# TimD1/vcfdist

Hardware: AMD Instinct MI355X
Metric: supercluster-alignments/sec (higher is better)
Workload: dtype int32; 1 GPU; wgs_synth; superclusters_per_gpu=1000000, span_dist=lognormal(median 20, sigma 1.2) clip [4,10000]

## Files before the change

vcfdist_amd/csrc/pr_api.hip:

```cpp
#include <hip/hip_runtime.h>
#include <hip/hip_ext.h>
#include <dlfcn.h>

#include <algorithm>
#include <atomic>
#include <chrono>
#include <cstdarg>
#include <cstdio>
#include <cstdlib>
#include <cstring>
#include <condition_variable>
#include <deque>
#include <functional>
#include <mutex>
#include <string>
#include <thread>
#include <tuple>
#include <unordered_map>
#include <unordered_set>
#include <vector>

#include "../../include/vcfdist_pr.h"
#include "pr_device.h"
#include "pr_plan.h"
// ... 935 lines not shown
    for (int k = 0; k < 2; k++)
        if (hipEventCreateWithFlags(&h->ev_cred[k], hipEventDisableTiming) != hipSuccess) return fail(nullptr, VPR_ERR_DEVICE, "hipEventCreate failed");
    if (const char *e = getenv("VPR_LONG_LT")) { const int v = atoi(e); if (v >= 64 && v <= 2048) h->long_lt = v; }
    memset(&h->dB, 0, sizeof(h->dB));
    memset(&h->timing, 0, sizeof(h->timing));
    const char *prio_map = exp_getenv("VPR_STREAM_PRIO");
    if (prio_map && strlen(prio_map) != size_t(N_CLASSES + 5)) prio_map = nullptr;
    if (hipSetDevice(cfg->device) != hipSuccess) { delete h; return fail(nullptr, VPR_ERR_DEVICE, "hipSetDevice failed"); }
    int prio_lo = 0, prio_hi = 0;
    (void)hipDeviceGetStreamPriorityRange(&prio_lo, &prio_hi);
    auto prio_of = [&](int idx, int dflt) { return !prio_map ? dflt : (prio_map[idx] == 'h' ? prio_hi : (prio_map[idx] == 'l' ? prio_lo : (prio_hi + prio_lo) / 2)); };
    if (hipStreamCreateWithPriority(&h->stream, exp_getenv("VPR_MAIN_BLOCKING") ? hipStreamDefault : hipStreamNonBlocking, prio_of(N_CLASSES + 4, (prio_hi + prio_lo) / 2)) != hipSuccess) {
        delete h;
        return fail(nullptr, VPR_ERR_DEVICE, "hipStreamCreate failed");
    }
    {
        size_t free_b = 0, total_b = 0;
        if (hipMemGetInfo(&free_b, &total_b) != hipSuccess) { delete h; return fail(nullptr, VPR_ERR_DEVICE, "hipMemGetInfo failed"); }
        h->dev_total = int64_t(total_b);
        h->tie_scratch_max = std::max<int64_t>(h->dev_total / 16, int64_t(64) << 20);
        h->lad_arena_max = std::max<int64_t>(h->dev_total / 8, int64_t(64) << 20);
    }
    if (const char *e = exp_getenv("VPR_STREAM_PAD")) {
        static std::atomic<int> n_handles{0};
        const int me = n_handles.fetch_add(1);
        const char *p = e;
        for (int i = 0; i < me && p; i++) { p = strchr(p, ','); if (p) p++; }
        if (p) {
            const int n_lo = atoi(p);
            const char *c = strchr(p, ':');
// ... 351 lines not shown
                h->res_dev = base; h->res_bytes = off;
            }
        }
    }
    if ((rc = dev_alloc(h, &R.tally, 6))) return rc;
    R.max_qual = h->cfg.max_qual;
    R.credit_threshold = h->cfg.credit_threshold;
    R.phase_threshold = h->cfg.phase_threshold;
    h->tie_list_cap = int32_t(std::min<size_t>(std::max<size_t>(na, 4096), size_t(1) << 20));
    if ((rc = dev_alloc(h, &h->d_tie_list, size_t(h->tie_list_cap)))) return rc;
    if ((rc = dev_alloc(h, &h->d_tie_cnt, 8))) return rc;
    if ((rc = dev_alloc(h, &h->d_tie_ndec, TIE_DEC_SLOTS))) return rc;
    const size_t n_fail = 4 * na + na / 16 + 1024, n_slots = 2 + 4 * LadderCtx::N_SLOTS;
    if ((rc = dev_alloc(h, &h->d_fail, n_fail))) return rc;
    if ((rc = dev_alloc(h, &h->d_cnt, n_slots))) return rc;
    {
        void *pf = nullptr, *pc = nullptr, *pl = nullptr, *pt = nullptr;
        { int rc_pin = pin_alloc(h, &pf, n_fail * sizeof(int32_t)); if (rc_pin) return rc_pin; }
        { int rc_pin = pin_alloc(h, &pc, n_slots * sizeof(int32_t)); if (rc_pin) return rc_pin; }
        { int rc_pin = pin_alloc(h, &pl, size_t(h->tie_list_cap) * sizeof(int4)); if (rc_pin) return rc_pin; }
        { int rc_pin = pin_alloc(h, &pt, 32 * sizeof(int32_t)); if (rc_pin) return rc_pin; }
        h->hp_fail = static_cast<int32_t *>(pf);
        h->hp_cnt = static_cast<int32_t *>(pc);
        h->hp_tie_list = static_cast<int4 *>(pl);
        h->hp_tie_cnt = static_cast<int32_t *>(pt);
        h->hp_flag = h->hp_tie_cnt + 8;
        memset(h->hp_cnt, 0, n_slots * sizeof(int32_t));
        memset(h->hp_tie_cnt, 0, 32 * sizeof(int32_t));
    }

// ... 313 lines not shown
    }
    double phase_ms[6] = {0, 0, 0, 0, 0, 0};
    void phase(int k) { phase_ms[k] = std::chrono::duration<double, std::milli>(std::chrono::steady_clock::now() - call0).count(); }
    void lapx(const char *what) {
        if (h->debug) fprintf(stderr, "[vpr] execute %-34s %8.3f ms\n", what,
                              std::chrono::duration<double, std::milli>(std::chrono::steady_clock::now() - wall0).count());
    }

    void post_flag(int idx, hipStream_t ks) {
        flag_exp[idx] = ++h->flag_seq;
        hipLaunchKernelGGL(k_flag, dim3(1), dim3(1), 0, ks, h->hp_flag + idx, flag_exp[idx]);
        const hipError_t e = hipGetLastError();
        if (e != hipSuccess && launch_err == hipSuccess) launch_err = e;
    }
    hipError_t launch_err = hipSuccess;
    int64_t zl_wave0 = 0, zl_rows = 0;

    int idle_check(int64_t idle_polls, std::chrono::steady_clock::time_point since) {
        if (launch_err != hipSuccess) return fail(h, VPR_ERR_DEVICE, "kernel launch failed: %s", hipGetErrorString(launch_err));
        if (idle_polls % 2048) return VPR_OK;
        hipStream_t ss[] = {h->stream, h->cls_stream[0], h->cls_stream[1], h->cls_stream[2], h->cls_stream[3], h->cls_stream[4],
                            h->cls_stream[5], h->cls_stream[6], h->cls_stream[7],
                            h->tie_stream[0], h->tie_stream[1], h->tie_stream[2], h->tie_stream[3]};
        bool busy = false;
        for (hipStream_t s_ : ss) {
            const hipError_t e = hipStreamQuery(s_);
            if (e != hipSuccess && e != hipErrorNotReady) return fail(h, VPR_ERR_DEVICE, "stream error while waiting for a round: %s", hipGetErrorString(e));
            busy = busy || e == hipErrorNotReady;
        }
        const double idle_s = std::chrono::duration<double>(std::chrono::steady_clock::now() - since).count();
// ... 407 lines not shown
            }
        }
        return VPR_OK;
    }

    int enqueue_part(const Plan &P, const int32_t *d_work, int64_t off, int32_t cnt, int lv, hipStream_t ks,
                            int slot, int64_t fail_off, bool long_part, int64_t part_cells, int64_t part_in,
                            int64_t part_dense, int dtag_override = -1, int phases = 7,
                            const int32_t *n_dev = nullptr, int32_t n_all = 0, int tag_or = 0) {
        const int W = LV_WINDOW[lv], C = W / 64, tag = LV_TAG[lv] | tag_or;
        const bool q16 = lv <= LV_Q16, zero = lv == LV_Z;
        const int dtag = dtag_override >= 0 ? dtag_override : tag;
        const int32_t *list = d_work + off;
        int32_t *a_i32 = reinterpret_cast<int32_t *>(P.arena);
        PathEnt *a_path = reinterpret_cast<PathEnt *>(P.arena);
        vpr_launch_stat ls;
        memset(&ls, 0, sizeof(ls));
        ls.threads = q16 ? 16 : 64; ls.cells_per_thread = q16 ? 1 : C; ls.n_units = cnt;
        ls.cells = part_cells;
        ls.cells_dense = part_dense;
        ls.bytes_algorithmic = ls.cells + part_in;
        int rc = VPR_OK;
        if (phases & 1) {
        if (zero) {
            ls.bytes_algorithmic = 36 * zl_rows;
            ls.cells = 8 * zl_rows;
        }
        cells_touched += ls.cells;
        const bool save = lv == LV_C1 && !tag_or && fwd_save_delta != 0;
        RestoreJob *rjobs = nullptr;
// ... 7 lines not shown
                const auto it = tie_early.find(P.work[size_t(off) + size_t(k)]);
                if (it == tie_early.end() || it->second.plan != &h->plan0 || (it->second.mode != 1 && it->second.mode != 3) ||
                    it->second.pos < tie_resident->work_off || it->second.pos >= tie_resident->work_off + tie_resident->n_long) { restore = false; break; }
                const AlnDesc od = plan_desc(h, h->plan0, size_t(it->second.pos)), nd = plan_desc(h, P, size_t(off) + size_t(k));
                if (od.band_pad != LV_TAG[LV_C1] || od.pitch[0] != nd.pitch[0] || od.pitch[1] != nd.pitch[1] ||
                    od.mat_off[1] + int64_t(od.pitch[1]) * od.Lt > h->save_bytes) { restore = false; break; }
                rjobs[k] = RestoreJob{{od.mat_off[0], od.mat_off[1]}, od.blo_off};
            }
        }
        rc = timed(1, ls, ks, restore ? "k_restore_stripe" : band_fwd_name(lv), [&] {
            if (zero)
                hipExtLaunchKernelGGL(k_zero_lane, dim3((cnt + 63) / 64), dim3(64), h->zl_lds_bytes, ks, own_a, own_b, 0, h->d_descs, list, cnt,
                                      h->d_zl_hdr + zl_wave0, h->d_zl_in, h->d_zl_log, h->d_outs, a_path,
                                      (h->cfg.flags & VPR_CFG_KEEP_PATHS) ? 1 : 0, h->d_d1_hdr ? h->d1_max_rows : 0, h->lane_prio_rows);
            else if (q16)
                hipLaunchKernelGGL(k_fwd_q16, dim3((cnt + 3) / 4), dim3(64), 0, ks, h->dB, h->d_descs, list, cnt,
                                   P.arena, a_i32, h->d_outs, n_dev);
            else if (restore)
                hipLaunchKernelGGL(k_restore_stripe, dim3(cnt), dim3(256), 0, ks, h->d_descs, list, rjobs, h->plan0.arena,
                                   int64_t(reinterpret_cast<intptr_t>(h->d_save) - reinterpret_cast<intptr_t>(h->plan0.arena)), P.arena, a_i32);
            else if (save)
                hipLaunchKernelGGL(k_fwd_stripe_save, dim3(cnt), dim3(64), 0, ks, h->dB, h->d_descs, list, P.arena, a_i32, h->d_outs,
                                   fwd_save_delta);
            else
                hipLaunchKernelGGL(band_fwd_kernel(lv), dim3(cnt), dim3(lv >= LV_C4 ? W : 64), 0,
                                   ks, h->dB, h->d_descs, list, P.arena, a_i32, h->d_outs);
            hipLaunchKernelGGL(k_fwd_band_finish, dim3((cnt + 255) / 256), dim3(256), 0, ks, list, cnt, h->d_outs, tag, n_dev);
        }, zero);
        if (rc) return rc;
        n_fwd++;
        {
            const int32_t nc = n_dev ? n_all : cnt;
            if (zero && h->d_d1_blk) ordered_fails(list, nc, h->d_fail + fail_off, h->d_cnt + slot, n_dev, ks);
            else
            hipLaunchKernelGGL(k_collect_fails, dim3((nc + 255) / 256), dim3(256), 0, ks, list, nc, h->d_outs,
                               h->d_fail + fail_off, h->d_cnt + slot, zero ? 1 : 0, n_dev);
            hipLaunchKernelGGL(k_publish_fails, dim3(zero ? 1 : std::min((nc + 255) / 256, 1024)), dim3(256), 0, ks,
                               h->d_fail + fail_off, h->d_cnt + slot, h->hp_fail + fail_off, h->hp_cnt + slot, zero ? 0 : 1);
        }
        HIPCHK(h, hipEventRecord(h->ev_slot[slot], ks));
        }
        if ((phases & 2) && !zero) {
        ls.bytes_algorithmic = ls.cells;
        rc = timed(2, ls, ks, band_bwd_name(lv), [&] {
            if (q16)
                hipLaunchKernelGGL(k_bwd_q16, dim3((cnt + 3) / 4), dim3(64), 0, ks, h->dB, h->d_descs, list, cnt,
                                   P.arena, a_i32, h->d_outs, tag, dtag, n_dev);
            else
                hipLaunchKernelGGL(band_bwd_kernel(lv), dim3(cnt), dim3(lv >= LV_C4 ? W : 64), 0,
                                   ks, h->dB, h->d_descs, list, P.arena, a_i32, h->d_outs, tag);
        });
        if (rc) return rc;
        }
        if (!(phases & 4)) return rc;
        const bool wave_walk = !q16 && (long_part || cnt < 2048);
        int64_t walk_rows_sum = 0;
        if (lv == LV_C1 && !h->seq_walk)
            for (int32_t k = 0; k < cnt && walk_rows_sum <= WSEG_MAX_ROWS; k++) walk_rows_sum += plan_desc(h, P, size_t(off) + size_t(k)).Lt;
        const bool seg_walk = lv == LV_C1 && !h->seq_walk && walk_rows_sum <= WSEG_MAX_ROWS;
        const bool row_walk = lv == LV_C1 && (wave_walk || seg_walk);
        vpr_launch_stat ws_;
        memset(&ws_, 0, sizeof(ws_));
        ws_.threads = q16 ? 16 : 64; ws_.n_units = cnt; ws_.cells_per_thread = 2;
        if (q16) {
            if (!zero) rc = timed(3, ws_, ks, "k_walk_q16", [&] {
                hipLaunchKernelGGL(k_walk_q16, dim3((cnt + 3) / 4), dim3(64), 0, ks, h->dB, h->d_descs, list, cnt,
                                   P.arena, a_i32, h->d_outs, a_path, tag, dtag, n_dev);
            });
            if (rc) return rc;
            ws_.cells_per_thread = 3;
            if (zero) ws_.bytes_algorithmic = 20 * zl_rows;
            if (zero) rc = timed(3, ws_, ks, "k_zero_tail", [&] {
                hipLaunchKernelGGL(k_zero_tail, dim3((cnt + 63) / 64), dim3(64), 0, ks, h->dB, h->d_descs, list, cnt, h->d_zl_hdr + zl_wave0,
                                   h->d_zl_in, h->d_zl_log, h->d_outs, a_path, (h->cfg.flags & VPR_CFG_KEEP_PATHS) ? 1 : 0, h->d_secs,
                                   h->d_fp_table, h->d_jobs, h->d_njobs, h->jobs_cap, tag, h->lane_prio_rows);
            });
            else if (cnt <= CREDIT_WAVE_MAX && !n_dev) rc = timed(3, ws_, ks, "k_credit<wave>", [&] {
                hipLaunchKernelGGL(k_credit<true>, dim3(cnt), dim3(64), 0, ks, h->dB, h->d_descs, list, cnt,
                                   h->d_outs, a_path, h->d_secs, h->d_fp_table, h->d_jobs, h->d_njobs,
                                   h->jobs_cap, dtag, tag, n_dev);
            });
            else {
                static const int head_max = [] { const char *e = exp_getenv("VPR_CREDIT_HEAD"); return e ? atoi(e) : 4096; }();
                const int32_t head = (n_dev && h->d_d1_blk && cnt > 2 * head_max) ? head_max : 0;
                if (head > 0) {
                    vpr_launch_stat wh_ = ws_;
                    wh_.n_units = head;
                    rc = timed(3, wh_, ks, "k_credit<wave>", [&] {
                        hipLaunchKernelGGL(k_credit<true>, dim3(head), dim3(64), 0, ks, h->dB, h->d_descs, list, head,
                                           h->d_outs, a_path, h->d_secs, h->d_fp_table, h->d_jobs, h->d_njobs,
                                           h->jobs_cap, dtag, tag, n_dev, 0);
                    });
                    if (rc) return rc;
                }
                rc = timed(3, ws_, ks, "k_credit<lane>", [&] {
                    hipLaunchKernelGGL(k_credit<false>, dim3((cnt - head + 63) / 64), dim3(64), 0, ks, h->dB, h->d_descs,
                                       list, cnt, h->d_outs, a_path, h->d_secs, h->d_fp_table, h->d_jobs,
                                       h->d_njobs, h->jobs_cap, dtag, tag, n_dev, int(head));
                });
            }
        } else if (row_walk) {
            static const int wseg_min_rows = [] { const char *e = exp_getenv("VPR_WSEG_MIN_ROWS"); return e ? atoi(e) : 2048; }();
            int32_t n_seg = cnt;
            if (seg_walk && long_part && wseg_min_rows > 0) {
                n_seg = 0;
                while (n_seg < cnt && plan_desc(h, P, size_t(off) + size_t(n_seg)).Lt >= wseg_min_rows) n_seg++;
            }
            if (!seg_walk || n_seg < cnt) {
                const int32_t k0 = seg_walk ? n_seg : 0;
                vpr_launch_stat wr_ = ws_;
                wr_.n_units = cnt - k0;
                rc = timed(3, wr_, ks, "k_walk_rows", [&] {
                    hipLaunchKernelGGL(k_walk_rows, dim3(cnt - k0), dim3(64), 0, ks, h->dB, h->d_descs, list + k0, cnt - k0,
// ... 482 lines not shown
            const int32_t *short_list = P0.d_work + ch.work_off + n_long;
            if (n_short > 0 && !inplace) {
                for (int ph = 1; ph <= 4; ph <<= 1) {
                    if ((rc = enqueue_part(P0, P0.d_work, ch.work_off + n_long, n_short, P0.lv, s_short, 1, n_long, false,
                                           ch.part_cells[1], ch.part_in[1], ch.part_dense[1], -1, ph))) return rc;
                    if (ph == 1) post_flag(1, s_short);
                    if (ph == 2 && (rc = collect_part(1, short_list, n_short, s_short))) return rc;
                }
            }
            if (inplace) {
                zl_wave0 = h->zl_wave0[ci];
                zl_rows = ch.part_rows[1];
                const int32_t *n_dev = h->d_cnt + 1;
                const int ztag = LV_TAG[LV_Z];
                HIPCHK(h, hipMemsetAsync(h->d_cnt + SLOT_IP, 0, 4, s_short));
                const bool d1 = h->d_d1_hdr != nullptr && cap_ip <= h->d1_wave_cap * 64;
                const int32_t n_all1 = n_short + n_short / 16 + 64;
                if (d1) HIPCHK(h, hipMemsetAsync(h->d_d1_info + 2, 0, 4, s_short));
                hipStream_t s_cred = h->side_credit ? h->cls_stream[7] : s_short;
                for (int ph = 1; ph <= 4; ph <<= 1) {
                    if (ph != 4 || s_cred == s_short) {
                        if ((rc = enqueue_part(P0, P0.d_work, ch.work_off + n_long, n_short, LV_Z, s_short, 1, n_long, false,
                                               ch.part_cells[1], ch.part_in[1], ch.part_dense[1], -1, ph))) return rc;
                        if (d1 && (rc = enqueue_d1(h->d_fail + n_long, n_dev, cap_ip, n_all1, s_short, ph, ztag))) return rc;
                    }
                    if (ph == 1 && s_cred != s_short) {
                        HIPCHK(h, hipEventRecord(h->ev_cred[0], s_short));
                        HIPCHK(h, hipStreamWaitEvent(s_cred, h->ev_cred[0], 0));
                        if ((rc = enqueue_part(P0, P0.d_work, ch.work_off + n_long, n_short, LV_Z, s_cred, 1, n_long, false,
                                               ch.part_cells[1], ch.part_in[1], ch.part_dense[1], -1, 4))) return rc;
                        if (d1 && (rc = enqueue_d1(h->d_fail + n_long, n_dev, cap_ip, n_all1, s_cred, 4, ztag))) return rc;
                        HIPCHK(h, hipEventRecord(h->ev_cred[1], s_cred));
                    }
                    if (ph == 4 && s_cred != s_short) HIPCHK(h, hipStreamWaitEvent(s_short, h->ev_cred[1], 0));
                    if ((rc = d1 ? enqueue_part(P0, h->d_d1_fail, 0, cap_ip, LV_Q16, s_short, SLOT_IP, foff_ip, false, 0, 0, 0,
                                                ztag, ph, h->d_d1_info + 2, std::min<int32_t>(h->d1_fail_cap, n_all1 + n_all1 / 64 + 64))
                                 : enqueue_part(P0, h->d_fail, n_long, cap_ip, LV_Q16, s_short, SLOT_IP, foff_ip, false, 0, 0, 0,
                                                ztag, ph, n_dev, n_all1))) return rc;
                    if (ph == 1) post_flag(1, s_short);
                    if (ph == 2 && (rc = collect_part(1, short_list, n_short, s_short))) return rc;
                }
            }
            if (n_long > 0) {
                const int lv = P0.lv <= LV_Q16 ? LONG_LV : P0.lv;
                for (int ph = 1; ph <= 4; ph <<= 1) {
                    fwd_save_delta = (ph == 1 && lv == LV_C1 && h->d_save) ? int64_t(reinterpret_cast<intptr_t>(h->d_save) - reinterpret_cast<intptr_t>(P0.arena)) : 0;
                    rc = enqueue_part(P0, P0.d_work, ch.work_off, n_long, lv, s_long, 0, 0, true, ch.part_cells[0],
                                      ch.part_in[0], ch.part_dense[0], -1, ph);
                    fwd_save_delta = 0;
                    if (rc) return rc;
                    if (ph == 1) {
                        post_flag(0, s_long);
                        if (lv == LV_C1) {
// ... 483 lines not shown
```

vcfdist_amd/csrc/pr_host.h:

```cpp
#ifndef PR_HOST_H_
#define PR_HOST_H_
#include <hip/hip_runtime.h>
#include <hip/hip_ext.h>

#include <algorithm>
#include <atomic>
#include <chrono>
#include <cstdarg>
#include <cstdio>
#include <cstdlib>
#include <cstring>
#include <condition_variable>
#include <deque>
#include <functional>
#include <mutex>
#include <string>
#include <thread>
#include <tuple>
#include <unordered_map>
#include <unordered_set>
#include <vector>

#include "../../include/vcfdist_pr.h"
#include "pr_device.h"
// ... 254 lines not shown
    uint8_t *d_arena = nullptr; int64_t arena_bytes = 0;
    LadderCtx lad[4];
    hipEvent_t ev_slot[2 + 4 * LadderCtx::N_SLOTS] = {};
    hipStream_t tie_stream[4] = {nullptr, nullptr, nullptr, nullptr};
    hipEvent_t ev_tie2[2] = {nullptr, nullptr};
    hipEvent_t ev_side[2] = {nullptr, nullptr};
    hipEvent_t ev_tie[2] = {nullptr, nullptr};
    std::vector<std::pair<std::vector<int32_t>, uint8_t *>> resident;
    int64_t res0_off = 0; int32_t res0_cnt = 0;
    Section *d_secs = nullptr; int64_t n_secs_cap = 0;
    int32_t *d_fp[4] = {nullptr, nullptr, nullptr, nullptr};
    int32_t **d_fp_table = nullptr;
    EdJob *d_jobs = nullptr; int32_t jobs_cap = 0; int32_t *d_njobs = nullptr;
    uint32_t *d_err = nullptr;
    int32_t *d_fail = nullptr, *d_cnt = nullptr;
    int4 *d_tie_list = nullptr, *hp_tie_list = nullptr; int32_t tie_list_cap = 0;
    int32_t *hp_flag = nullptr; int32_t flag_seq = 0;
    int32_t *d_tie_cnt = nullptr, *hp_tie_cnt = nullptr;
    hipEvent_t ev_spec = nullptr;
    TieJob *hp_tie_jobs = nullptr; size_t tie_jobs_cap = 0;
    int4 *d_tie_dec = nullptr; int64_t tie_dec_cap = 0;
    int32_t *d_tie_ndec = nullptr;
    std::vector<int32_t> plan0_pos;
    ZlWave *d_zl_hdr = nullptr; uint32_t *d_zl_in = nullptr; uint4 *d_zl_log = nullptr;
    std::vector<int64_t> zl_wave0;
    ZlWave *d_d1_hdr = nullptr; uint32_t *d_d1_in = nullptr; uint4 *d_d1_log = nullptr; int32_t *d_d1_fail = nullptr, *d_d1_info = nullptr;
    int32_t *d_d1_blk = nullptr;
    hipEvent_t ev_offsets = nullptr;
    hipEvent_t ev_cred[2] = {nullptr, nullptr};
    bool side_credit = true;
// ... 125 lines not shown
```

vcfdist_amd/csrc/pr_kernels.hip:

```cpp
#include <hip/hip_runtime.h>
#include <stdint.h>

#include "../../include/vcfdist_pr.h"
#include "pr_device.h"
#include "pr_scan.h"

__device__ __forceinline__ bool fwd_allow(int f) { return !(f & PV) || (f & PE); }
__device__ __forceinline__ bool bwd_allow(int f) { return !(f & PV) || (f & PB); }

__global__ void __launch_bounds__(256) k_prep_scof(DevBatch B) {
    __shared__ int64_t s_off[257];
    const int which = blockIdx.y;
    const int64_t *off = which < 4 ? B.hap_off[which] : B.ref_off;
    int32_t *out = which < 4 ? B.sc_hap[which] : B.sc_ref;
    const int sc0 = blockIdx.x * 256, m = min(256, B.n_sc - sc0);
    for (int i = threadIdx.x; i <= m; i += 256) s_off[i] = off[sc0 + i];
    __syncthreads();
    const int64_t beg = s_off[0], end = s_off[m];
    for (int64_t g = beg + threadIdx.x; g < end; g += 256) {
        int lo = 0, hi = m;
        while (hi - lo > 1) {
            const int mid = (lo + hi) >> 1;
            if (s_off[mid] <= g) lo = mid; else hi = mid;
        }
// ... 1106 lines not shown
        bool in_q = (hi == ri) ? false : bool(qflv & PV);
        if (hi == qi && consumes) in_q = in_q && !(qflv & PB);
        const bool sync = !in_t && !in_q && !ins_loc && tr == qr && (mv & (F_MAT | F_SWP | F_SUB));
        if (n >= d.path_cap) { status |= VPR_ST_ERR_LIMIT; ok = false; break; }
        if (lead) path[n] = PathEnt{uint32_t(qri) | (uint32_t(hi) << 31),
                                    uint32_t(ti) | (uint32_t(sync) << 31) | (edit << 30), qr, tr};
        n++;
    }
    if (lead) O.path_len = int32_t(n);
    if (!ok) { if (lead) { atomicOr(&O.status, status); O.n_sec = 0; } return; }
    if (WAVE) asm volatile("s_waitcnt vmcnt(0)" ::: "memory");

    credit_walk<WAVE>(B, d, O, a, path, n, status, secs, fp_group, jobs, n_jobs, jobs_cap, lead);
}

template <bool WAVE>
__global__ void __launch_bounds__(64) k_credit(DevBatch B, const AlnDesc *__restrict__ descs,
                       const int32_t *__restrict__ work, int n_work, AlnOut *__restrict__ outs,
                       const PathEnt *__restrict__ paths, Section *__restrict__ secs,
                       int32_t *const *__restrict__ fp_group,
                       EdJob *__restrict__ jobs, int32_t *__restrict__ n_jobs, int32_t jobs_cap, int my_w, int ok_tag,
                       const int32_t *__restrict__ n_dev, int first = 0) {
    if (n_dev) n_work = min(n_work, *n_dev);
    const int wi = first + (WAVE ? int(blockIdx.x) : int(blockIdx.x * blockDim.x + threadIdx.x));
    if (wi >= n_work) return;
    if (WAVE) __builtin_amdgcn_s_setprio(2);
    const int a = work[wi];
    if (a < 0) return;
    const AlnDesc d = descs[a];
    AlnOut &O = outs[a];
    if (d.band_pad != my_w || (my_w > 0 ? O.band_ok != ok_tag : O.band_ok < 0)) return;
    if (O.status & (VPR_ST_ERR_NO_PTR | VPR_ST_ERR_LIMIT)) return;
    const bool lead = !WAVE || (threadIdx.x & 63) == 0;
    credit_walk<WAVE>(B, d, O, a, paths + d.path_off, int64_t(O.path_len), 0u, secs, fp_group, jobs, n_jobs, jobs_cap, lead);
}

__global__ void k_finalize(const AlnDesc *__restrict__ descs, int n_aln, const AlnOut *__restrict__ outs,
                           const Section *__restrict__ secs, int32_t *const *__restrict__ fp_group, DevResults R,
                           const uint8_t *__restrict__ sc_limit, const uint8_t *__restrict__ alias) {
    const int a = blockIdx.x * blockDim.x + threadIdx.x;
    if (a >= n_aln) return;
    const AlnDesc d = descs[a];
    const AlnOut O = outs[a];
    uint32_t status = O.status;
    int src_i = -1;
    {
        const int b = alias[d.sc], q = d.aln >> 1, t = d.aln & 1;
        const int si = ((b & 1) ? 0 : q) * 2 + ((b & 2) ? 0 : t);
        if (si != d.aln) src_i = si;
// ... 260 lines not shown
```

vcfdist_amd/csrc/pr_mem.hip:

```cpp
#include "pr_host.h"

namespace {
std::string g_create_err;
}
const char *vpr_create_error() { return g_create_err.c_str(); }

int fail(vpr_handle *h, int code, const char *fmt, ...) {
    char buf[512];
    va_list ap;
    va_start(ap, fmt);
    vsnprintf(buf, sizeof(buf), fmt, ap);
    va_end(ap);
    if (h) h->err = buf; else g_create_err = buf;
    return code;
}


inline void slow_call(vpr_handle *h, const char *what, const char *site, size_t bytes, double dt) {
    if (h && h->stall_log && dt > 5.0) fprintf(stderr, "[vpr] slow host call: %s (%zu bytes) at %s: %.1f ms\n", what, bytes, site, dt);
}
const char *exp_getenv(const char *name) {
#ifdef VPR_EXPERIMENTS
    return getenv(name);
#else
// ... 266 lines not shown
        if (h->want0 > 0 && h->lad[k].arena_bytes > 0) h->lad_hw[k] = double(h->lad[k].arena_bytes) / double(h->want0);
        LadderCtx keep;
        for (int e = 0; e < 2; e++) {
            keep.tie_scratch[e] = h->lad[k].tie_scratch[e]; keep.tie_scratch_bytes[e] = h->lad[k].tie_scratch_bytes[e];
            keep.tie_first[e] = h->lad[k].tie_first[e];
        }
        h->lad[k] = keep;
    }
    for (auto &b : h->parked) h->dev_cache.push_back(b);
    h->parked.clear();
    h->resident.clear();
    h->res0_cnt = 0;
    h->d_ed_scratch = nullptr; h->ed_scratch_ints = 0;
    h->d_tie_list = nullptr; h->hp_tie_list = nullptr; h->tie_list_cap = 0; h->d_tie_cnt = nullptr; h->hp_tie_cnt = nullptr;
    h->hp_tie_jobs = nullptr; h->tie_jobs_cap = 0;
    h->d_tie_dec = nullptr; h->tie_dec_cap = 0; h->d_tie_ndec = nullptr; h->plan0_pos.clear();
    h->d_zl_hdr = nullptr; h->d_zl_in = nullptr; h->d_zl_log = nullptr; h->zl_wave0.clear();
    h->d_d1_hdr = nullptr; h->d_d1_in = nullptr; h->d_d1_log = nullptr; h->d_d1_fail = nullptr; h->d_d1_info = nullptr; h->d_d1_blk = nullptr;
    h->d1_in_cap = h->d1_log_cap = 0; h->d1_wave_cap = h->d1_fail_cap = 0;
    h->uploaded = h->executed = false;
}

int64_t books_free(int64_t reported_free, int64_t total) { return dev_books().books_free(reported_free, total); }
```

vcfdist_amd/csrc/pr_q16.hip:

```cpp
#ifndef PR_Q16_HIP_
#define PR_Q16_HIP_

#define Q_W 16
#define Q_K 4

__global__ void k_prep_q16(DevBatch B, int which, int64_t n_pos) {
    const int64_t g = int64_t(blockIdx.x) * blockDim.x + threadIdx.x;
    if (g >= n_pos) return;
    const int slot = which < 2 ? which : (which < 4 ? -1 : which - 2);
    const int64_t *off = slot >= 0 ? B.hap_off[slot] : B.ref_off;
    const int lo = (slot >= 0 ? B.sc_hap[slot] : B.sc_ref)[g];
    const int64_t beg = off[lo];
    const int64_t gm1 = g > beg ? g - 1 : beg;
    if (which < 2) {
        const int2 k = B.fk_q[which][g];
        B.fk4_q[which][g] = make_int4(k.x, k.y, B.hap_ptr[which][g], B.vs_hap[which][gm1]);
    } else if (which < 4) {
        const int h = which - 2;
        const int2 k = B.fk_r[h][g];
        B.fk4_r[h][g] = make_int4(k.x, k.y, int32_t(g - beg), B.vs_ref[h][gm1]);
    } else {
        const int f = g > beg ? int(B.hap_flag[slot][g - 1]) : 0;
        const int at = (!(f & PV) || (f & PE)) ? 1 : 0;
        B.tk[which - 4][g] = make_int2(B.hap_ptr[slot][g],
// ... 61 lines not shown
    asm volatile(
        "s_nop 1\n\t"
        MP_STEP("row_shr:1") MP_STEP("row_shr:2") MP_STEP("row_shr:4") MP_STEP("row_shr:8")
        "s_nop 0"
        : "+v"(Aq), "+v"(Bq), "+v"(Ar), "+v"(Br), "=&v"(tq), "=&v"(tr));
#undef MP_STEP
    a.A = (Aq >= MP_OFF) ? Aq - MP_OFF : S_NEG; a.B = (Bq < 0) ? -1 : Bq;
    b.A = (Ar >= MP_OFF) ? Ar - MP_OFF : S_NEG; b.B = (Br < 0) ? -1 : Br;
}

__device__ __forceinline__ int wave_max4(int v) {
    return max(max(__builtin_amdgcn_readlane(v, 0), __builtin_amdgcn_readlane(v, 16)),
               max(__builtin_amdgcn_readlane(v, 32), __builtin_amdgcn_readlane(v, 48)));
}

__global__ void __launch_bounds__(64) k_fwd_q16(DevBatch B, const AlnDesc *__restrict__ descs,
                                                const int32_t *__restrict__ work, int n_work,
                                                uint8_t *__restrict__ ws, int32_t *__restrict__ blo_all,
                                                AlnOut *__restrict__ outs, const int32_t *__restrict__ n_dev) {
    if (n_dev) n_work = min(n_work, *n_dev);
    if (int(blockIdx.x) * 4 >= n_work) return;
    const int lane = threadIdx.x, gl = lane & 15, gbase = lane & 48;
    const int wi = int(blockIdx.x) * 4 + (lane >> 4);
    const int a_ = work[min(wi, n_work - 1)];
    const bool live = wi < n_work && a_ >= 0;
    const int a = max(a_, 0);
    const AlnDesc *dp = descs + a;
    const int Lq = dp->Lq, Lr = dp->Lr, Lt = live ? dp->Lt : 0;
    const int qs = dp->qs, ts = dp->ts;
    const int64_t q_off = dp->q_off, r_off = dp->r_off;
    const int Lp[2] = {Lq, Lr};
    const int2 *tk = (ts == 2 ? B.tk[0] : B.tk[1]) + dp->t_off;
    const uint16_t *tjp = (ts == 2 ? B.tj[0] : B.tj[1]) + dp->t_off;
    const int32_t *r2q = (qs == 0 ? B.ref_ptr[0] : B.ref_ptr[1]) + r_off;
    const int4 *fk[2] = {(qs == 0 ? B.fk4_q[0] : B.fk4_q[1]) + q_off, (qs == 0 ? B.fk4_r[0] : B.fk4_r[1]) + r_off};
    auto load_k = [&](int p, int idx) -> int4 { return fk[p][idx]; };
    const int4 *cand[2] = {(qs == 0 ? B.cand_q[0] : B.cand_q[1]) + q_off, (qs == 0 ? B.cand_r[0] : B.cand_r[1]) + r_off};
    const int4 *cand2[2] = {(qs == 0 ? B.cand2_q[0] : B.cand2_q[1]) + q_off, (qs == 0 ? B.cand2_r[0] : B.cand2_r[1]) + r_off};
// ... 190 lines not shown
            cbQ = nbQ; cbR = nbR;
            origin(s + 1 + 16 + gl, nbQ, nbR);
        }
    }
    const int dq = grp_get(gbase, Lq - 1 - dlo[0], Dp[0], D_INF);
    const int dr = grp_get(gbase, Lr - 1 - dlo[1], Dp[1], D_INF);
    int em = exit_min, dummy = D_INF;
    row_prefix_min2(em, dummy);
    if (live && gl == 15) {
        outs[a].dist_q = dq;
        outs[a].dist_r = dr;
        outs[a].exit_min = em;
    }
}

__global__ void __launch_bounds__(64) k_bwd_q16(DevBatch B, const AlnDesc *__restrict__ descs,
                                                const int32_t *__restrict__ work, int n_work,
                                                uint8_t *__restrict__ ws, const int32_t *__restrict__ blo_all,
                                                AlnOut *__restrict__ outs, int tag, int dtag,
                                                const int32_t *__restrict__ n_dev) {
    if (n_dev) n_work = min(n_work, *n_dev);
    if (int(blockIdx.x) * 4 >= n_work) return;
    const int lane = threadIdx.x, gl = lane & 15, gbase = lane & 48;
    const int wi = int(blockIdx.x) * 4 + (lane >> 4);
    const int a_ = work[min(wi, n_work - 1)];
    const bool live = wi < n_work && a_ >= 0;
    const int a = max(a_, 0);
    const AlnDesc *dp = descs + a;
    const bool on = live && outs[a].band_ok == tag && dp->band_pad == dtag;
    const int Lq = dp->Lq, Lr = dp->Lr, Lt = on ? dp->Lt : 0;
    const int qs = dp->qs;
    const int Lp[2] = {Lq, Lr};
    const int32_t *bk[2] = {(qs == 0 ? B.bk_q[0] : B.bk_q[1]) + dp->q_off, (qs == 0 ? B.bk_r[0] : B.bk_r[1]) + dp->r_off};
    uint32_t *mat = reinterpret_cast<uint32_t *>(ws + dp->mat_off[0]);
    const int2 *blo2 = reinterpret_cast<const int2 *>(blo_all + dp->blo_off);
    const int end_plane = outs[a].end_plane;
    const int nstr = (Lt + Q_K - 1) / Q_K;
    const int smax = wave_max4(nstr);
    if (smax == 0) return;
// ... 132 lines not shown
            mat[s * 32 + 16 + col] = oacc[1];
        }
        if (act) { plo[0] = lo[0]; plo[1] = lo[1]; }
        lo[0] = nlo[0]; lo[1] = nlo[1];
        bkc[0] = bkn[0]; bkc[1] = bkn[1];
        fw[0] = fwn[0]; fw[1] = fwn[1];
        if ((s & 15) == 0 && s > 0) {
            cbQ = lbQ; cbR = lbR;
            load_chunk(((s - 1) & ~15) - 16, lbQ, lbR);
        }
    }
    if (on && gl == 15) outs[a].beg_plane = (sc1[0] >= 0) ? VPR_PLANE_QUERY : VPR_PLANE_REF;
    if (on && tie_used) { atomicOr(&outs[a].status, VPR_ST_SWAP_TIE); outs[a].band_ok = TIE_MARK(tag); atomicAdd(&outs[a].n_sec, int(tie_used)); }
}

__global__ void __launch_bounds__(64) k_walk_q16(DevBatch B, const AlnDesc *__restrict__ descs,
                                                 const int32_t *__restrict__ work, int n_work,
                                                 const uint8_t *__restrict__ ws, const int32_t *__restrict__ blo_all,
                                                 AlnOut *__restrict__ outs, PathEnt *__restrict__ paths, int tag, int dtag,
                                                 const int32_t *__restrict__ n_dev) {
    if (n_dev) n_work = min(n_work, *n_dev);
    if (int(blockIdx.x) * 4 >= n_work) return;
    const int lane = threadIdx.x, gl = lane & 15, gbase = lane & 48;
    const int wi = int(blockIdx.x) * 4 + (lane >> 4);
    const int a_ = work[min(wi, n_work - 1)];
    const bool live = wi < n_work && a_ >= 0;
    const int a = max(a_, 0);
    const AlnDesc *dp = descs + a;
    const bool on = live && outs[a].band_ok == tag && dp->band_pad == dtag;
    const int Lq = dp->Lq, Lr = dp->Lr, Lt = on ? dp->Lt : 0;
    const int qs = dp->qs, ts = dp->ts;
    const int path_cap = dp->path_cap;
    const int2 *wq = (qs == 0 ? B.wk_q[0] : B.wk_q[1]) + dp->q_off;
    const int2 *wr = (qs == 0 ? B.wk_r[0] : B.wk_r[1]) + dp->r_off;
    const int2 *wt = (ts == 2 ? B.wk_t[0] : B.wk_t[1]) + dp->t_off;
    const int insmask = ((1 << qs) | (1 << ts)) << 8;
    const uint32_t *mat = reinterpret_cast<const uint32_t *>(ws + dp->mat_off[0]);
    const int2 *blo2 = reinterpret_cast<const int2 *>(blo_all + dp->blo_off);
    PathEnt *path = paths + dp->path_off;
// ... 105 lines not shown
        lo[0] = nlo[0]; lo[1] = nlo[1];
        pp[0] = ppn[0]; pp[1] = ppn[1];
        cq = cqn; cr = crn;
        if (((s + 1) & 15) == 0) {
            cbQ = nbQ; cbR = nbR;
            load_chunk(s + 1 + 16, nbQ, nbR);
        }
    }
    if (on && gl == 0) {
        outs[a].path_len = n;
        if (!ok) outs[a].n_sec = 0;
        if (status) atomicOr(&outs[a].status, status);
    }
}

#endif
```

Before: 202.9 million supercluster-alignments/s.

## Add optional atomic-ticket persistent scheduling to q16 and credit kernels

Wraps the q16 forward, backward and walk kernels and the lane credit kernel in a loop. When the VPR_TICKET_WGS env var is set, each wave draws the next work group from a global atomic ticket, and the grid is capped at a resident count computed from occupancy. This targets launch and tail imbalance on lognormal-sized alignments. It also adds min-waves-per-EU launch bounds, which are active regardless of the env var and may force register limits or spills.

```diff
diff --git a/vcfdist_amd/csrc/pr_api.hip b/vcfdist_amd/csrc/pr_api.hip
--- a/vcfdist_amd/csrc/pr_api.hip
+++ b/vcfdist_amd/csrc/pr_api.hip
@@ -973,6 +973,19 @@
         delete h;
         return fail(nullptr, VPR_ERR_DEVICE, "hipStreamCreate failed");
     }
+    if (const char *e = getenv("VPR_TICKET_WGS")) {
+        const void *fn[vpr_handle::TK_N] = {reinterpret_cast<const void *>(k_fwd_q16), reinterpret_cast<const void *>(k_bwd_q16),
+                                            reinterpret_cast<const void *>(k_walk_q16), reinterpret_cast<const void *>(k_credit<false>)};
+        const bool aut = strcmp(e, "auto") == 0;
+        int n_cu = 0;
+        if (aut && hipDeviceGetAttribute(&n_cu, hipDeviceAttributeMultiprocessorCount, cfg->device) != hipSuccess) { delete h; return fail(nullptr, VPR_ERR_DEVICE, "hipDeviceGetAttribute failed"); }
+        for (int k = 0; k < vpr_handle::TK_N; k++) {
+            int per_cu = 0;
+            if (!aut) h->ticket_wgs[k] = std::max(0, atoi(e));
+            else if (hipOccupancyMaxActiveBlocksPerMultiprocessor(&per_cu, fn[k], 64, 0) != hipSuccess || per_cu <= 0) { delete h; return fail(nullptr, VPR_ERR_DEVICE, "hipOccupancyMaxActiveBlocksPerMultiprocessor failed"); }
+            else h->ticket_wgs[k] = n_cu * per_cu;
+        }
+    }
     {
         size_t free_b = 0, total_b = 0;
         if (hipMemGetInfo(&free_b, &total_b) != hipSuccess) { delete h; return fail(nullptr, VPR_ERR_DEVICE, "hipMemGetInfo failed"); }
@@ -1354,6 +1367,7 @@
     const size_t n_fail = 4 * na + na / 16 + 1024, n_slots = 2 + 4 * LadderCtx::N_SLOTS;
     if ((rc = dev_alloc(h, &h->d_fail, n_fail))) return rc;
     if ((rc = dev_alloc(h, &h->d_cnt, n_slots))) return rc;
+    if ((rc = dev_alloc(h, &h->d_ticket, size_t(vpr_handle::TK_N)))) return rc;
     {
         void *pf = nullptr, *pc = nullptr, *pl = nullptr, *pt = nullptr;
         { int rc_pin = pin_alloc(h, &pf, n_fail * sizeof(int32_t)); if (rc_pin) return rc_pin; }
@@ -1697,6 +1711,7 @@
         if (e != hipSuccess && launch_err == hipSuccess) launch_err = e;
     }
     hipError_t launch_err = hipSuccess;
+    bool part_tickets = false;
     int64_t zl_wave0 = 0, zl_rows = 0;
 
     int idle_check(int64_t idle_polls, std::chrono::steady_clock::time_point since) {
@@ -2134,6 +2149,9 @@
         const int32_t *list = d_work + off;
         int32_t *a_i32 = reinterpret_cast<int32_t *>(P.arena);
         PathEnt *a_path = reinterpret_cast<PathEnt *>(P.arena);
+        const bool tickets = part_tickets && n_dev && q16 && !zero;
+        auto tk_word = [&](int k) -> int32_t * { return tickets && h->ticket_wgs[k] > 0 ? h->d_ticket + k : nullptr; };
+        auto tk_grid = [&](int k, int32_t n_grp) { return dim3(unsigned(tk_word(k) ? std::min<int32_t>(n_grp, h->ticket_wgs[k]) : n_grp)); };
         vpr_launch_stat ls;
         memset(&ls, 0, sizeof(ls));
         ls.threads = q16 ? 16 : 64; ls.cells_per_thread = q16 ? 1 : C; ls.n_units = cnt;
@@ -2171,8 +2189,8 @@
                                       h->d_zl_hdr + zl_wave0, h->d_zl_in, h->d_zl_log, h->d_outs, a_path,
                                       (h->cfg.flags & VPR_CFG_KEEP_PATHS) ? 1 : 0, h->d_d1_hdr ? h->d1_max_rows : 0, h->lane_prio_rows);
             else if (q16)
-                hipLaunchKernelGGL(k_fwd_q16, dim3((cnt + 3) / 4), dim3(64), 0, ks, h->dB, h->d_descs, list, cnt,
-                                   P.arena, a_i32, h->d_outs, n_dev);
+                hipLaunchKernelGGL(k_fwd_q16, tk_grid(vpr_handle::TK_FWD, (cnt + 3) / 4), dim3(64), 0, ks, h->dB, h->d_descs, list, cnt,
+                                   P.arena, a_i32, h->d_outs, n_dev, tk_word(vpr_handle::TK_FWD));
             else if (restore)
                 hipLaunchKernelGGL(k_restore_stripe, dim3(cnt), dim3(256), 0, ks, h->d_descs, list, rjobs, h->plan0.arena,
                                    int64_t(reinterpret_cast<intptr_t>(h->d_save) - reinterpret_cast<intptr_t>(h->plan0.arena)), P.arena, a_i32);
@@ -2201,8 +2219,8 @@
         ls.bytes_algorithmic = ls.cells;
         rc = timed(2, ls, ks, band_bwd_name(lv), [&] {
             if (q16)
-                hipLaunchKernelGGL(k_bwd_q16, dim3((cnt + 3) / 4), dim3(64), 0, ks, h->dB, h->d_descs, list, cnt,
-                                   P.arena, a_i32, h->d_outs, tag, dtag, n_dev);
+                hipLaunchKernelGGL(k_bwd_q16, tk_grid(vpr_handle::TK_BWD, (cnt + 3) / 4), dim3(64), 0, ks, h->dB, h->d_descs, list, cnt,
+                                   P.arena, a_i32, h->d_outs, tag, dtag, n_dev, tk_word(vpr_handle::TK_BWD));
             else
                 hipLaunchKernelGGL(band_bwd_kernel(lv), dim3(cnt), dim3(lv >= LV_C4 ? W : 64), 0,
                                    ks, h->dB, h->d_descs, list, P.arena, a_i32, h->d_outs, tag);
@@ -2221,8 +2239,8 @@
         ws_.threads = q16 ? 16 : 64; ws_.n_units = cnt; ws_.cells_per_thread = 2;
         if (q16) {
             if (!zero) rc = timed(3, ws_, ks, "k_walk_q16", [&] {
-                hipLaunchKernelGGL(k_walk_q16, dim3((cnt + 3) / 4), dim3(64), 0, ks, h->dB, h->d_descs, list, cnt,
-                                   P.arena, a_i32, h->d_outs, a_path, tag, dtag, n_dev);
+                hipLaunchKernelGGL(k_walk_q16, tk_grid(vpr_handle::TK_WALK, (cnt + 3) / 4), dim3(64), 0, ks, h->dB, h->d_descs, list, cnt,
+                                   P.arena, a_i32, h->d_outs, a_path, tag, dtag, n_dev, tk_word(vpr_handle::TK_WALK));
             });
             if (rc) return rc;
             ws_.cells_per_thread = 3;
@@ -2251,9 +2269,9 @@
                     if (rc) return rc;
                 }
                 rc = timed(3, ws_, ks, "k_credit<lane>", [&] {
-                    hipLaunchKernelGGL(k_credit<false>, dim3((cnt - head + 63) / 64), dim3(64), 0, ks, h->dB, h->d_descs,
+                    hipLaunchKernelGGL(k_credit<false>, tk_grid(vpr_handle::TK_CREDIT, (cnt - head + 63) / 64), dim3(64), 0, ks, h->dB, h->d_descs,
                                        list, cnt, h->d_outs, a_path, h->d_secs, h->d_fp_table, h->d_jobs,
-                                       h->d_njobs, h->jobs_cap, dtag, tag, n_dev, int(head));
+                                       h->d_njobs, h->jobs_cap, dtag, tag, n_dev, int(head), tk_word(vpr_handle::TK_CREDIT));
                 });
             }
         } else if (row_walk) {
@@ -2766,6 +2784,7 @@
                 const int32_t *n_dev = h->d_cnt + 1;
                 const int ztag = LV_TAG[LV_Z];
                 HIPCHK(h, hipMemsetAsync(h->d_cnt + SLOT_IP, 0, 4, s_short));
+                HIPCHK(h, hipMemsetAsync(h->d_ticket, 0, vpr_handle::TK_N * 4, s_short));
                 const bool d1 = h->d_d1_hdr != nullptr && cap_ip <= h->d1_wave_cap * 64;
                 const int32_t n_all1 = n_short + n_short / 16 + 64;
                 if (d1) HIPCHK(h, hipMemsetAsync(h->d_d1_info + 2, 0, 4, s_short));
@@ -2785,10 +2804,12 @@
                         HIPCHK(h, hipEventRecord(h->ev_cred[1], s_cred));
                     }
                     if (ph == 4 && s_cred != s_short) HIPCHK(h, hipStreamWaitEvent(s_short, h->ev_cred[1], 0));
+                    part_tickets = true;
                     if ((rc = d1 ? enqueue_part(P0, h->d_d1_fail, 0, cap_ip, LV_Q16, s_short, SLOT_IP, foff_ip, false, 0, 0, 0,
                                                 ztag, ph, h->d_d1_info + 2, std::min<int32_t>(h->d1_fail_cap, n_all1 + n_all1 / 64 + 64))
                                  : enqueue_part(P0, h->d_fail, n_long, cap_ip, LV_Q16, s_short, SLOT_IP, foff_ip, false, 0, 0, 0,
                                                 ztag, ph, n_dev, n_all1))) return rc;
+                    part_tickets = false;
                     if (ph == 1) post_flag(1, s_short);
                     if (ph == 2 && (rc = collect_part(1, short_list, n_short, s_short))) return rc;
                 }
diff --git a/vcfdist_amd/csrc/pr_host.h b/vcfdist_amd/csrc/pr_host.h
--- a/vcfdist_amd/csrc/pr_host.h
+++ b/vcfdist_amd/csrc/pr_host.h
@@ -292,6 +292,9 @@
     EdJob *d_jobs = nullptr; int32_t jobs_cap = 0; int32_t *d_njobs = nullptr;
     uint32_t *d_err = nullptr;
     int32_t *d_fail = nullptr, *d_cnt = nullptr;
+    enum { TK_FWD = 0, TK_BWD, TK_WALK, TK_CREDIT, TK_N };
+    int32_t *d_ticket = nullptr;
+    int32_t ticket_wgs[TK_N] = {0, 0, 0, 0};
     int4 *d_tie_list = nullptr, *hp_tie_list = nullptr; int32_t tie_list_cap = 0;
     int32_t *hp_flag = nullptr; int32_t flag_seq = 0;
     int32_t *d_tie_cnt = nullptr, *hp_tie_cnt = nullptr;
diff --git a/vcfdist_amd/csrc/pr_kernels.hip b/vcfdist_amd/csrc/pr_kernels.hip
--- a/vcfdist_amd/csrc/pr_kernels.hip
+++ b/vcfdist_amd/csrc/pr_kernels.hip
@@ -1144,16 +1144,26 @@
     credit_walk<WAVE>(B, d, O, a, path, n, status, secs, fp_group, jobs, n_jobs, jobs_cap, lead);
 }
 
+__device__ __forceinline__ int draw_ticket(int32_t *ticket) {
+    int t = 0;
+    if ((threadIdx.x & 63) == 0) t = atomicAdd(ticket, 1);
+    return __builtin_amdgcn_readfirstlane(t);
+}
+
+__device__ __forceinline__ int group_lane() {
+    int lane = threadIdx.x;
+    asm volatile("" : "+v"(lane));
+    return lane;
+}
+
+template <class T> __device__ __forceinline__ T group_arg(T p) { asm volatile("" : "+s"(p)); return p; }
+
 template <bool WAVE>
-__global__ void __launch_bounds__(64) k_credit(DevBatch B, const AlnDesc *__restrict__ descs,
-                       const int32_t *__restrict__ work, int n_work, AlnOut *__restrict__ outs,
+__device__ __forceinline__ void credit_entry(const int wi, const DevBatch &B, const AlnDesc *__restrict__ descs,
+                       const int32_t *__restrict__ work, AlnOut *__restrict__ outs,
                        const PathEnt *__restrict__ paths, Section *__restrict__ secs,
                        int32_t *const *__restrict__ fp_group,
-                       EdJob *__restrict__ jobs, int32_t *__restrict__ n_jobs, int32_t jobs_cap, int my_w, int ok_tag,
-                       const int32_t *__restrict__ n_dev, int first = 0) {
-    if (n_dev) n_work = min(n_work, *n_dev);
-    const int wi = first + (WAVE ? int(blockIdx.x) : int(blockIdx.x * blockDim.x + threadIdx.x));
-    if (wi >= n_work) return;
+                       EdJob *__restrict__ jobs, int32_t *__restrict__ n_jobs, const int32_t jobs_cap, const int my_w, const int ok_tag) {
     if (WAVE) __builtin_amdgcn_s_setprio(2);
     const int a = work[wi];
     if (a < 0) return;
@@ -1163,6 +1173,32 @@
     if (O.status & (VPR_ST_ERR_NO_PTR | VPR_ST_ERR_LIMIT)) return;
     const bool lead = !WAVE || (threadIdx.x & 63) == 0;
     credit_walk<WAVE>(B, d, O, a, paths + d.path_off, int64_t(O.path_len), 0u, secs, fp_group, jobs, n_jobs, jobs_cap, lead);
+}
+
+template <bool WAVE>
+__global__ void __launch_bounds__(64, WAVE ? 1 : 5) k_credit(DevBatch B, const AlnDesc *__restrict__ descs,
+                       const int32_t *__restrict__ work, int n_work, AlnOut *__restrict__ outs,
+                       const PathEnt *__restrict__ paths, Section *__restrict__ secs,
+                       int32_t *const *__restrict__ fp_group,
+                       EdJob *__restrict__ jobs, int32_t *__restrict__ n_jobs, int32_t jobs_cap, int my_w, int ok_tag,
+                       const int32_t *__restrict__ n_dev, int first = 0, int32_t *__restrict__ ticket = nullptr) {
+    if (n_dev) n_work = min(n_work, *n_dev);
+    if constexpr (WAVE) {
+        const int wi = first + int(blockIdx.x);
+        if (wi >= n_work) return;
+        credit_entry<true>(wi, B, descs, work, outs, paths, secs, fp_group, jobs, n_jobs, jobs_cap, my_w, ok_tag);
+    } else {
+        for (int grp = int(blockIdx.x);;) {
+            if (ticket) grp = draw_ticket(ticket);
+            const int w0 = first + grp * 64;
+            if (w0 >= n_work) return;
+            const int wi = w0 + group_lane();
+            if (wi < n_work)
+                credit_entry<false>(wi, B, group_arg(descs), group_arg(work), group_arg(outs), group_arg(paths), group_arg(secs),
+                                    group_arg(fp_group), group_arg(jobs), group_arg(n_jobs), jobs_cap, my_w, ok_tag);
+            if (!ticket) return;
+        }
+    }
 }
 
 __global__ void k_finalize(const AlnDesc *__restrict__ descs, int n_aln, const AlnOut *__restrict__ outs,
diff --git a/vcfdist_amd/csrc/pr_mem.hip b/vcfdist_amd/csrc/pr_mem.hip
--- a/vcfdist_amd/csrc/pr_mem.hip
+++ b/vcfdist_amd/csrc/pr_mem.hip
@@ -304,7 +304,7 @@
     h->d_ed_scratch = nullptr; h->ed_scratch_ints = 0;
     h->d_tie_list = nullptr; h->hp_tie_list = nullptr; h->tie_list_cap = 0; h->d_tie_cnt = nullptr; h->hp_tie_cnt = nullptr;
     h->hp_tie_jobs = nullptr; h->tie_jobs_cap = 0;
-    h->d_tie_dec = nullptr; h->tie_dec_cap = 0; h->d_tie_ndec = nullptr; h->plan0_pos.clear();
+    h->d_tie_dec = nullptr; h->tie_dec_cap = 0; h->d_tie_ndec = nullptr; h->d_ticket = nullptr; h->plan0_pos.clear();
     h->d_zl_hdr = nullptr; h->d_zl_in = nullptr; h->d_zl_log = nullptr; h->zl_wave0.clear();
     h->d_d1_hdr = nullptr; h->d_d1_in = nullptr; h->d_d1_log = nullptr; h->d_d1_fail = nullptr; h->d_d1_info = nullptr; h->d_d1_blk = nullptr;
     h->d1_in_cap = h->d1_log_cap = 0; h->d1_wave_cap = h->d1_fail_cap = 0;
diff --git a/vcfdist_amd/csrc/pr_q16.hip b/vcfdist_amd/csrc/pr_q16.hip
--- a/vcfdist_amd/csrc/pr_q16.hip
+++ b/vcfdist_amd/csrc/pr_q16.hip
@@ -99,14 +99,12 @@
                max(__builtin_amdgcn_readlane(v, 32), __builtin_amdgcn_readlane(v, 48)));
 }
 
-__global__ void __launch_bounds__(64) k_fwd_q16(DevBatch B, const AlnDesc *__restrict__ descs,
-                                                const int32_t *__restrict__ work, int n_work,
-                                                uint8_t *__restrict__ ws, int32_t *__restrict__ blo_all,
-                                                AlnOut *__restrict__ outs, const int32_t *__restrict__ n_dev) {
-    if (n_dev) n_work = min(n_work, *n_dev);
-    if (int(blockIdx.x) * 4 >= n_work) return;
-    const int lane = threadIdx.x, gl = lane & 15, gbase = lane & 48;
-    const int wi = int(blockIdx.x) * 4 + (lane >> 4);
+__device__ __forceinline__ void fwd_q16_group(const int grp, const DevBatch &B, const AlnDesc *__restrict__ descs,
+                                              const int32_t *__restrict__ work, const int n_work,
+                                              uint8_t *__restrict__ ws, int32_t *__restrict__ blo_all,
+                                              AlnOut *__restrict__ outs) {
+    const int lane = group_lane(), gl = lane & 15, gbase = lane & 48;
+    const int wi = grp * 4 + (lane >> 4);
     const int a_ = work[min(wi, n_work - 1)];
     const bool live = wi < n_work && a_ >= 0;
     const int a = max(a_, 0);
@@ -327,15 +325,26 @@
     }
 }
 
-__global__ void __launch_bounds__(64) k_bwd_q16(DevBatch B, const AlnDesc *__restrict__ descs,
+__global__ void __launch_bounds__(64, 4) k_fwd_q16(DevBatch B, const AlnDesc *__restrict__ descs,
                                                 const int32_t *__restrict__ work, int n_work,
-                                                uint8_t *__restrict__ ws, const int32_t *__restrict__ blo_all,
-                                                AlnOut *__restrict__ outs, int tag, int dtag,
-                                                const int32_t *__restrict__ n_dev) {
+                                                uint8_t *__restrict__ ws, int32_t *__restrict__ blo_all,
+                                                AlnOut *__restrict__ outs, const int32_t *__restrict__ n_dev,
+                                                int32_t *__restrict__ ticket = nullptr) {
     if (n_dev) n_work = min(n_work, *n_dev);
-    if (int(blockIdx.x) * 4 >= n_work) return;
-    const int lane = threadIdx.x, gl = lane & 15, gbase = lane & 48;
-    const int wi = int(blockIdx.x) * 4 + (lane >> 4);
+    for (int grp = int(blockIdx.x);;) {
+        if (ticket) grp = draw_ticket(ticket);
+        if (grp * 4 >= n_work) return;
+        fwd_q16_group(grp, B, descs, work, n_work, ws, blo_all, outs);
+        if (!ticket) return;
+    }
+}
+
+__device__ __forceinline__ void bwd_q16_group(const int grp, const DevBatch &B, const AlnDesc *__restrict__ descs,
+                                              const int32_t *__restrict__ work, const int n_work,
+                                              uint8_t *__restrict__ ws, const int32_t *__restrict__ blo_all,
+                                              AlnOut *__restrict__ outs, const int tag, const int dtag) {
+    const int lane = group_lane(), gl = lane & 15, gbase = lane & 48;
+    const int wi = grp * 4 + (lane >> 4);
     const int a_ = work[min(wi, n_work - 1)];
     const bool live = wi < n_work && a_ >= 0;
     const int a = max(a_, 0);
@@ -498,15 +507,26 @@
     if (on && tie_used) { atomicOr(&outs[a].status, VPR_ST_SWAP_TIE); outs[a].band_ok = TIE_MARK(tag); atomicAdd(&outs[a].n_sec, int(tie_used)); }
 }
 
-__global__ void __launch_bounds__(64) k_walk_q16(DevBatch B, const AlnDesc *__restrict__ descs,
-                                                 const int32_t *__restrict__ work, int n_work,
-                                                 const uint8_t *__restrict__ ws, const int32_t *__restrict__ blo_all,
-                                                 AlnOut *__restrict__ outs, PathEnt *__restrict__ paths, int tag, int dtag,
-                                                 const int32_t *__restrict__ n_dev) {
+__global__ void __launch_bounds__(64, 7) k_bwd_q16(DevBatch B, const AlnDesc *__restrict__ descs,
+                                                const int32_t *__restrict__ work, int n_work,
+                                                uint8_t *__restrict__ ws, const int32_t *__restrict__ blo_all,
+                                                AlnOut *__restrict__ outs, int tag, int dtag,
+                                                const int32_t *__restrict__ n_dev, int32_t *__restrict__ ticket = nullptr) {
     if (n_dev) n_work = min(n_work, *n_dev);
-    if (int(blockIdx.x) * 4 >= n_work) return;
-    const int lane = threadIdx.x, gl = lane & 15, gbase = lane & 48;
-    const int wi = int(blockIdx.x) * 4 + (lane >> 4);
+    for (int grp = int(blockIdx.x);;) {
+        if (ticket) grp = draw_ticket(ticket);
+        if (grp * 4 >= n_work) return;
+        bwd_q16_group(grp, B, descs, work, n_work, ws, blo_all, outs, tag, dtag);
+        if (!ticket) return;
+    }
+}
+
+__device__ __forceinline__ void walk_q16_group(const int grp, const DevBatch &B, const AlnDesc *__restrict__ descs,
+                                               const int32_t *__restrict__ work, const int n_work,
+                                               const uint8_t *__restrict__ ws, const int32_t *__restrict__ blo_all,
+                                               AlnOut *__restrict__ outs, PathEnt *__restrict__ paths, const int tag, const int dtag) {
+    const int lane = group_lane(), gl = lane & 15, gbase = lane & 48;
+    const int wi = grp * 4 + (lane >> 4);
     const int a_ = work[min(wi, n_work - 1)];
     const bool live = wi < n_work && a_ >= 0;
     const int a = max(a_, 0);
@@ -642,4 +662,18 @@
     }
 }
 
+__global__ void __launch_bounds__(64, 7) k_walk_q16(DevBatch B, const AlnDesc *__restrict__ descs,
+                                                 const int32_t *__restrict__ work, int n_work,
+                                                 const uint8_t *__restrict__ ws, const int32_t *__restrict__ blo_all,
+                                                 AlnOut *__restrict__ outs, PathEnt *__restrict__ paths, int tag, int dtag,
+                                                 const int32_t *__restrict__ n_dev, int32_t *__restrict__ ticket = nullptr) {
+    if (n_dev) n_work = min(n_work, *n_dev);
+    for (int grp = int(blockIdx.x);;) {
+        if (ticket) grp = draw_ticket(ticket);
+        if (grp * 4 >= n_work) return;
+        walk_q16_group(grp, B, descs, work, n_work, ws, blo_all, outs, paths, tag, dtag);
+        if (!ticket) return;
+    }
+}
+
 #endif
```

New measurement: 195.2 million supercluster-alignments/s. 3.8% lower.
